# chorowski-lab/pytorch-asr

Hardware: AMD Instinct MI355X
Metric: CTC train-step frames/sec (higher is better)
Workload: dtype bf16; 1 GPU; WSJ mono-char CTC (egs/wsj/yamls/ctc.yaml shapes), DeepSpeech2 conv+4xBiLSTM-320 encoder + FSTDecoder, fwd+bwd+GradientClipping(clip 480000, skip 4.8e+06 = recipe x global_batch/16)+PolyakDecay+Adam, synthetic 40-dim x 1-channel x 1000-frame fbank; batch_per_gpu=768, global_batch=768, frames=1000, classes=49, parallelism=dp1, batch_norm=per-replica statistics, optimizer_steps=139, step_boundary=device: att_speech.fused_step (clip / skip decision + Adam, no read-back)

## Files before the change

### include/asr_amd.h

```cpp
#ifndef ASR_AMD_H
#define ASR_AMD_H

#include <stdint.h>

#ifdef __cplusplus
extern "C" {
#endif

enum {
    ASR_OK = 0,
    ASR_EINVAL = 1,
    ASR_EUNSUPPORTED = 2,
    ASR_ELAUNCH = 3
};

int asr_abi_version(void);

const char *asr_strerror(int code);

int64_t asr_lattice_fwbw_workspace_bytes(int T, int B, int C, int N);

int asr_lattice_fwbw_f32(const float *lp, int T, int B, int C,
                         const int32_t *lens,
                         const int32_t *src_in, const int32_t *il_in,
// ... 169 lines not shown
int64_t asr_conv7x7c32_workspace_bytes(void);
int asr_conv7x7c32_fwd_bf16(const void *x, const float *w, int B, int H, int W, int stride_h,
                            void *y, double *chan_sums, void *workspace, int64_t workspace_bytes,
                            void *stream);
int asr_conv7x7c32_bwd_data_bf16(const void *dy, const float *w, int B, int H, int W,
                                 int stride_h, void *dx, void *workspace,
                                 int64_t workspace_bytes, void *stream);
int asr_conv7x7c32_wgrad_bf16(const void *x, const void *dy, int B, int H, int W, int stride_h,
                              float *dw, void *workspace, int64_t workspace_bytes, void *stream);

int64_t asr_conv1_7x7s2_workspace_bytes(void);
int asr_conv1_7x7s2_fwd(const float *x, const float *w, int B, int T, int F, void *y,
                        double *chan_sums, void *workspace, int64_t workspace_bytes, void *stream);
int asr_conv1_7x7s2_wgrad(const float *x, const void *dy, int B, int T, int F, float *dw,
                          void *workspace, int64_t workspace_bytes, void *stream);

int64_t asr_conv1c_7x7s2_workspace_bytes(int cin);
int asr_conv1c_7x7s2_fwd(const float *x, const float *w, int B, int T, int F, int cin, void *y,
                         double *chan_sums, void *workspace, int64_t workspace_bytes, void *stream);
int asr_conv1c_7x7s2_wgrad(const float *x, const void *dy, int B, int T, int F, int cin,
                           float *dw, void *workspace, int64_t workspace_bytes, void *stream);

int asr_tcn_attention_step_f32(const float *eproj, const float *enc, const int32_t *enc_lens,
                               const float *filt, const float *glob, const float *w_score,
                               float b_score, float temperature,
                               const float *att_prev, const int32_t *parent,
                               int T, int B, int beam, int A, int Kf, int E,
                               float *att_new, float *context, void *stream);

int asr_tcn_attention_scan_fwd_f32(const float *eproj, const float *filt, const float *glob,
// ... 123 lines not shown
```

### pytorch-asr_amd/att_speech/_native.py

```python
import ctypes
import warnings
import os

import torch

_HERE = os.path.dirname(os.path.abspath(__file__))
LIB_PATH = os.environ.get(
    'ASR_AMD_LIB', os.path.join(os.path.dirname(_HERE), 'csrc', 'libasr_amd.so'))

ASR_OK, ASR_EINVAL, ASR_EUNSUPPORTED, ASR_ELAUNCH = 0, 1, 2, 3
ABI_VERSION = 24

_lib = None
EVENT_HOOK = None
_WARNED = {}

_vp, _i, _i64, _f = ctypes.c_void_p, ctypes.c_int, ctypes.c_int64, ctypes.c_float

_SIGNATURES = {
    'asr_abi_version': (ctypes.c_int, []),
    'asr_strerror': (ctypes.c_char_p, [_i]),
    'asr_lattice_fwbw_workspace_bytes': (_i64, [_i, _i, _i, _i]),
    'asr_lattice_fwbw_f32': (_i, [_vp, _i, _i, _i, _vp, _vp, _vp, _vp, _vp, _vp,
                                  _vp, _vp, _i, _i, _i, _i, _f, _vp, _vp, _vp,
# ... 9 lines not shown
    'asr_lattice_viterbi_workspace_bytes': (_i64, [_i, _i, _i]),
    'asr_lattice_forward_f32': (_i, [_vp, _i, _i, _i, _vp, _vp, _vp, _vp, _vp,
                                     _i, _i, _i, _f, _i, _vp, _vp, _vp, _i64,
                                     _vp]),
    'asr_log_softmax_fwd_f32': (_i, [_vp, _i64, _i, _vp, _vp]),
    'asr_log_softmax_bwd_f32': (_i, [_vp, _vp, _i64, _i, _vp, _vp]),
    'asr_sub_rowmax_f32': (_i, [_vp, _i, _i, _i, _vp, _vp, _vp, _vp, _vp]),
    'asr_argmax_rows_f32': (_i, [_vp, _i64, _i, _vp, _vp]),
    'asr_conv7x7c32_workspace_bytes': (_i64, []),
    'asr_conv7x7c32_fwd_bf16': (_i, [_vp, _vp, _i, _i, _i, _i, _vp, _vp, _vp, _i64, _vp]),
    'asr_conv7x7c32_bwd_data_bf16': (_i, [_vp, _vp, _i, _i, _i, _i, _vp, _vp, _i64, _vp]),
    'asr_conv7x7c32_wgrad_bf16': (_i, [_vp, _vp, _i, _i, _i, _i, _vp, _vp, _i64, _vp]),
    'asr_conv1_7x7s2_workspace_bytes': (_i64, []),
    'asr_conv1_7x7s2_fwd': (_i, [_vp, _vp, _i, _i, _i, _vp, _vp, _vp, _i64, _vp]),
    'asr_conv1_7x7s2_wgrad': (_i, [_vp, _vp, _i, _i, _i, _vp, _vp, _i64, _vp]),
    'asr_conv1c_7x7s2_workspace_bytes': (_i64, [_i]),
    'asr_conv1c_7x7s2_fwd': (_i, [_vp, _vp, _i, _i, _i, _i, _vp, _vp, _vp, _i64, _vp]),
    'asr_conv1c_7x7s2_wgrad': (_i, [_vp, _vp, _i, _i, _i, _i, _vp, _vp, _i64, _vp]),
    'asr_log_softmax_shift_fwd_f32': (_i, [_vp, _i, _i, _i, _vp, _vp, _vp, _vp, _vp]),
    'asr_log_softmax_shift_bwd_f32': (_i, [_vp, _vp, _vp, _i64, _i, _vp, _vp]),
    'asr_sum_leading_f32': (_i, [_vp, _i, _i64, _vp, _vp]),
    'asr_adam_chunk_elems': (_i, []),
    'asr_grad_sumsq_partials_f32': (_i, [_vp, _i64, _vp, _i, _vp]),
    'asr_adam_clip_step_f32': (_i, [_vp, _i, _vp, _vp, _vp, _vp, _i, _vp, _f, _f, _f, _f, _f, _f, _f,
                                    _vp, _vp, _vp, _vp]),
    'asr_adam_clip_step_ex_f32': (_i, [_vp, _i, _vp, _vp, _vp, _vp, _i, _vp, _f, _f, _f, _f, _f, _f, _f,
                                       _vp, _vp, _vp, _vp, _vp]),
    'asr_nonfinite_flag_f32': (_i, [_vp, _i, _vp, _vp]),
    'asr_noise_chunk_elems': (_i, []),
    'asr_gaussian_noise_f32': (_i, [_vp, _i, ctypes.c_uint64, ctypes.c_uint32, ctypes.c_uint64, _i, _i, _vp]),
# ... 1120 lines not shown
    if cin == 1:
        nbytes = L.asr_conv1_7x7s2_workspace_bytes()
        ws = torch.empty(nbytes, dtype=torch.uint8, device=x.device)
        check(L.asr_conv1_7x7s2_wgrad(_p(x), _p(dy), B, T, F, _p(dw), _p(ws), nbytes, _stream()),
              'asr_conv1_7x7s2_wgrad')
    else:
        nbytes = L.asr_conv1c_7x7s2_workspace_bytes(cin)
        if nbytes < 0:
            raise NotImplementedError('conv1_wgrad: %d input channels' % cin)
        ws = torch.empty(nbytes, dtype=torch.uint8, device=x.device)
        check(L.asr_conv1c_7x7s2_wgrad(_p(x), _p(dy), B, T, F, cin, _p(dw), _p(ws), nbytes, _stream()),
              'asr_conv1c_7x7s2_wgrad')
    return dw


def split_bf16(x, hi=None, lo=None):
    x = _dev(x, torch.float32, 'x')
    if hi is None:
        hi = torch.empty(x.shape, dtype=torch.bfloat16, device=x.device)
        lo = torch.empty(x.shape, dtype=torch.bfloat16, device=x.device)
        rows, cols, ldx, ldh, ldl = 1, x.numel(), x.numel(), x.numel(), x.numel()
    else:
        if x.dim() != 2 or hi.shape != x.shape or lo.shape != x.shape or x.stride(1) != 1 \
                or hi.stride(1) != 1 or lo.stride(1) != 1 or hi.dtype != torch.bfloat16 or lo.dtype != torch.bfloat16:
            raise ValueError('split_bf16: x, hi, lo must be [rows, cols] with a dense last dimension')
        rows, cols = x.shape
        ldx, ldh, ldl = x.stride(0), hi.stride(0), lo.stride(0)
    check(lib().asr_split_bf16_f32(_p(x), rows, cols, ldx, _p(hi), ldh, _p(lo), ldl, _stream()),
          'asr_split_bf16_f32')
    return hi, lo
# ... 65 lines not shown
```

### pytorch-asr_amd/att_speech/modules/encoders/deep_speech_2.py

```python
import warnings
from collections import OrderedDict

import torch
from torch import nn

from att_speech.modules.encoders.base_encoder import BaseEncoder
from att_speech.modules.encoders.encoder_utils import (
    BatchRNN, Normalization, SequentialWithOptionalAttributes)


class DeepSpeech2(BaseEncoder):
    def __init__(self, sample_batch, conv_normalization='batch_norm',
                 conv_strides=[[2, 2], [2, 1]],
                 conv_kernel_sizes=[[41, 11], [21, 11]],
                 conv_num_features=[32, 32],
                 rnn_hidden_size=768, rnn_nb_layers=5, rnn_projection_size=0,
                 rnn_type=nn.LSTM, rnn_dropout=0.0, rnn_residual=False,
                 rnn_normalization='batch_norm', rnn_subsample=None, **kwargs):
        super(DeepSpeech2, self).__init__(**kwargs)
        import os
        self.conv_bf16 = os.environ.get('ASR_CONV_BF16', '1') != '0'
        self.fused_bn = os.environ.get('ASR_FUSED_BN', '1') != '0'
        self.native_conv = os.environ.get('ASR_NATIVE_CONV', '1') != '0'
        if isinstance(rnn_type, str):
# ... 76 lines not shown
                                            c.dilation, c.groups)
            y = nn.functional.conv2d(
                x.to(torch.bfloat16), c.weight.to(torch.bfloat16),
                None if bias is None else bias.to(torch.bfloat16),
                c.stride, c.padding, c.dilation, c.groups)
            return y if keep_bf16 else y.float()

        def second_conv(x, with_bias=True):
            return run_conv(c2, x, with_bias)

        if fused:
            from att_speech.modules.encoders.native_bn import bn_hardtanh
            from att_speech.modules.encoders import native_conv
            c1 = conv[0]
            sums1 = sums2 = None
            if bf16 and self.native_conv and native_conv.first_supported(c1, features):
                x, sums1 = native_conv.conv1(features, c1)
            else:
                if bf16 and self.native_conv and not getattr(self, '_warned_conv1', False):
                    self._warned_conv1 = True
                    warnings.warn('DeepSpeech2: the first convolution is not a (1 or 3)->32 7x7 stride-(1,2) '
                                  'shape on gradient-free features csrc/conv.hip is built for; using '
                                  'torch / MIOpen for it')
                x = run_conv(c1, features, with_bias=False, keep_bf16=True)
            x = bn_hardtanh(x, conv[1].batch_norm, conv[2], out_bf16=bf16, conv_bias=c1.bias,
                            chan_sums=sums1)
            if bf16 and self.native_conv and native_conv.supported(c2, x):
                y2, sums2 = native_conv.conv7x7c32(x, c2)
            else:
                if bf16 and self.native_conv and not getattr(self, '_warned_conv', False):
                    self._warned_conv = True
                    warnings.warn('DeepSpeech2: the second convolution is not the 32->32 7x7 '
                                  'stride-(3,1) shape csrc/conv.hip is built for; using torch / MIOpen')
                y2 = run_conv(c2, x, with_bias=False, keep_bf16=True)
            x = bn_hardtanh(y2, conv[4].batch_norm, conv[5], time_major=True, conv_bias=c2.bias,
                            chan_sums=sums2, out_bf16=bf16 and self._rnn_takes_bf16(y2))
            return x.view(x.size(0), x.size(1), -1)
        if bf16:
            x = conv[5](conv[4](second_conv(conv[2](conv[1](conv[0](features))))))
        else:
            x = conv(features)
# ... 24 lines not shown
```

### pytorch-asr_amd/att_speech/modules/encoders/native_bn.py

```python
import torch
import torch.distributed as dist

from att_speech import _native

SYNC = {'on': False, 'group': None}


def _sync_active():
    return (SYNC['on'] and dist.is_available() and dist.is_initialized()
            and dist.get_world_size(SYNC['group']) > 1)


def _allreduce_sums(sums, n_local):
    buf = torch.cat([sums.reshape(-1), sums.new_tensor([n_local])])
    dist.all_reduce(buf, op=dist.ReduceOp.SUM, group=SYNC['group'])
    sums.copy_(buf[:-1].view_as(sums))
    return float(buf[-1])


class BNHardtanhFunction(torch.autograd.Function):
    @staticmethod
    def forward(ctx, x, gamma, beta, conv_bias, running_mean, running_var, training, momentum,
                eps, lo, hi, out_bf16, time_major, chan_sums=None, sync_counts=None):
        out, mean, invstd = _native.bn_act_fwd(
            x, gamma.detach(), beta.detach(), running_mean, running_var, training, momentum,
            eps, lo, hi, out_bf16=out_bf16, time_major=time_major,
            conv_bias=None if conv_bias is None else conv_bias.detach(), chan_sums=chan_sums)
        if sync_counts is not None and running_var is not None and momentum:
            nl, nt = sync_counts
            var = invstd.double().pow(-2) - eps
            running_var.add_((momentum * var * (nt / (nt - 1.0) - nl / (nl - 1.0))).float())
        ctx.has_cb = conv_bias is not None
        ctx.save_for_backward(x, gamma, beta, mean, invstd,
                              conv_bias if conv_bias is not None else gamma)
        ctx.cfg = (training, lo, hi, time_major)
        ctx.sync = training and _sync_active()
        return out

    @staticmethod
    def backward(ctx, dy):
        x, gamma, beta, mean, invstd, cb = ctx.saved_tensors
        training, lo, hi, time_major = ctx.cfg
        dx, dgamma, dbeta, dcb = _native.bn_act_bwd(
            x, gamma.detach(), beta.detach(), mean, invstd, training, lo, hi, dy,
            time_major=time_major, conv_bias=cb.detach() if ctx.has_cb else None,
            sync=_allreduce_sums if ctx.sync else None)
        return (dx, dgamma, dbeta, dcb) + (None,) * 11


def bn_hardtanh(x, bn, act, out_bf16=False, time_major=False, conv_bias=None, chan_sums=None):
    use_batch_stats = bn.training or bn.running_mean is None
    momentum = 0.0
    rm = rv = None
    if use_batch_stats and bn.training and bn.track_running_stats and bn.running_mean is not None:
        bn.num_batches_tracked.add_(1)
        momentum = bn.momentum if bn.momentum is not None else 1.0 / float(bn.num_batches_tracked)
        rm, rv = bn.running_mean, bn.running_var
    elif not use_batch_stats:
        rm, rv = bn.running_mean, bn.running_var
    if x.dtype != torch.bfloat16:
        x = x.float()
    sync_counts = None
    if use_batch_stats and bn.training and _sync_active():
        n_local = float(x.shape[0] * x.shape[2] * x.shape[3])
        if chan_sums is None:
            xd = x.double()
            chan_sums = torch.stack([xd.sum((0, 2, 3)), (xd * xd).sum((0, 2, 3))])
        else:
            chan_sums = chan_sums.clone()
        n_total = _allreduce_sums(chan_sums, n_local)
        chan_sums.mul_(n_local / n_total)
        sync_counts = (n_local, n_total)
    return BNHardtanhFunction.apply(x, bn.weight, bn.bias, conv_bias, rm, rv, use_batch_stats,
                                    momentum, bn.eps, float(act.min_val), float(act.max_val),
                                    out_bf16, time_major, chan_sums if use_batch_stats else None,
                                    sync_counts)
```

### pytorch-asr_amd/att_speech/modules/encoders/native_conv.py

```python
import torch

from att_speech import _native


def supported(conv, x):
    return (x.is_cuda and isinstance(conv, torch.nn.Conv2d) and conv.in_channels == 32
            and conv.out_channels == 32 and tuple(conv.kernel_size) == (7, 7)
            and tuple(conv.stride) == (3, 1) and tuple(conv.padding) == (0, 0)
            and tuple(conv.dilation) == (1, 1) and conv.groups == 1
            and x.dim() == 4 and x.size(2) >= 7 and 7 <= x.size(3) <= 48)


class Conv7x7C32Function(torch.autograd.Function):
    @staticmethod
    def forward(ctx, x, weight):
        x = x.to(torch.bfloat16).contiguous(memory_format=torch.channels_last)
        ctx.save_for_backward(x, weight)
        y, sums = _native.conv7x7c32_fwd(x, weight.detach(), 3, want_sums=True)
        ctx.mark_non_differentiable(sums)
        return y, sums

    @staticmethod
    def backward(ctx, dy, _dsums):
        x, weight = ctx.saved_tensors
        dx = dw = None
# ... 18 lines not shown

    @staticmethod
    def forward(ctx, x, weight):
        x = x.float().contiguous()
        ctx.save_for_backward(x, weight)
        y, sums = _native.conv1_fwd(x, weight.detach(), want_sums=True)
        ctx.mark_non_differentiable(sums)
        return y, sums

    @staticmethod
    def backward(ctx, dy, _dsums):
        x, weight = ctx.saved_tensors
        return None, (_native.conv1_wgrad(x, dy) if ctx.needs_input_grad[1] else None)


def conv1(features, conv):
    if features.size(1) == 1:
        return Conv1Function.apply(features[:, 0], conv.weight)
    return Conv1Function.apply(features.permute(0, 2, 3, 1), conv.weight)


def conv7x7c32(x, conv):
    return Conv7x7C32Function.apply(x, conv.weight)
```

### pytorch-asr_amd/csrc/bnact.hip

```cpp
#include "common.h"
#include "../../include/asr_amd.h"

namespace {

using namespace asr;

struct BnParams {
    const float *x;
    int B, C, HW, Wd;
    const float *gamma, *beta;
    const float *mean, *invstd;
    const float *shift;
    float lo, hi;
};

__global__ __launch_bounds__(256) void bn_stats_kernel(const float *x, const float *shift, int C, int HW, double *sums) {
    __shared__ float red[64];
    const int c = blockIdx.x, b = blockIdx.y;
    const float *p = x + ((size_t)b * C + c) * HW;
    const float sh0 = shift ? shift[c] : 0.f;
    float s = 0.f, q = 0.f;
    for (int i = threadIdx.x; i < HW; i += 256) {
        const float v = p[i] + sh0;
        s += v;
// ... 390 lines not shown
    const int C = p.C;
    NHWC8_THREAD_SETUP(p.P);
    float m[8], is[8], g[8], be[8], k1[8], k2[8], s[8], q[8];
#pragma unroll
    for (int i = 0; i < 8; ++i) {
        m[i] = p.mean[c0 + i] - (p.shift ? p.shift[c0 + i] : 0.f);
        is[i] = p.invstd[c0 + i]; g[i] = p.gamma[c0 + i]; be[i] = p.beta[c0 + i];
        k1[i] = MODE == 1 && training ? (float)(sums[2 * (c0 + i)] / n) : 0.f;
        k2[i] = MODE == 1 && training ? (float)(sums[2 * (c0 + i) + 1] / n) : 0.f;
        s[i] = q[i] = 0.f;
    }
    auto one = [&](int64_t pix, const F8 &v, const F8 &dv) {
        F8 o;
#pragma unroll
        for (int i = 0; i < 8; ++i) {
            const float xh = (v.v[i] - m[i]) * is[i];
            const float y = fmaf(xh, g[i], be[i]);
            const float d = (y > p.lo && y < p.hi) ? dv.v[i] : 0.f;
            if (MODE == 0) { s[i] += d; q[i] += d * xh; }
            else o.v[i] = g[i] * is[i] * (d - k1[i] - xh * k2[i]);
        }
        if (MODE == 1) store8(dx + pix * C + c0, o);
    };
    for (int64_t pix = (int64_t)blockIdx.x * 2 * PL + pl; pix < pend; pix += cstep) {
        if (pix + PL < pend) {
            const F8 v0 = load8(px + pix * C + c0), v1 = load8(px + (pix + PL) * C + c0);
            const F8 d0 = load8(dy + pix * C + c0), d1 = load8(dy + (pix + PL) * C + c0);
            one(pix, v0, d0);
            one(pix + PL, v1, d1);
        } else {
            one(pix, load8(px + pix * C + c0), load8(dy + pix * C + c0));
        }
    }
    if (MODE == 0) nhwc_block_atomics8(s, q, C, sums);
}
// ... 207 lines not shown
    return hipGetLastError() == hipSuccess ? ASR_OK : ASR_ELAUNCH;
}

extern "C" int asr_bn_act_bwd_phase_f32(const void *x, int x_bf16, const float *conv_bias, int B, int C, int H, int W,
                                  const float *gamma, const float *beta,
                                  const float *save_mean, const float *save_invstd,
                                  int channels_last,
                                  int training, float lo, float hi,
                                  const void *dy, int dy_bf16, int dy_time_major,
                                  void *dx, float *dgamma, float *dbeta, float *dconv_bias,
                                  void *workspace, int64_t workspace_bytes, int phase,
                                  double n_total, void *stream) {
    if (phase < 0 || phase > 2 || (phase == 2 && !(n_total >= 1.0))) return ASR_EINVAL;
    const bool do_reduce = phase != 2, do_apply = phase != 1;
    if (bad_shape(B, C, H, W) || !x || !gamma || !beta || !save_mean || !save_invstd || !dy ||
        !dx || !dgamma || !dbeta)
        return ASR_EINVAL;
    if (!workspace || workspace_bytes < asr_bn_act_workspace_bytes(C)) return ASR_EINVAL;
    hipStream_t s = (hipStream_t)stream;
    double *sums = (double *)workspace;
    const int HW = H * W;
    const dim3 grid(C, B);
    BnParams p;
    p.x = (const float *)x; p.B = B; p.C = C; p.HW = HW; p.Wd = W; p.gamma = gamma; p.beta = beta;
    p.mean = save_mean; p.invstd = save_invstd; p.shift = conv_bias; p.lo = lo; p.hi = hi;
    const double n = phase == 2 ? n_total : (double)B * HW;
    if (do_reduce)
        hipLaunchKernelGGL(zero_doubles_kernel, dim3((2 * C + 255) / 256), dim3(256), 0, s, sums, 2 * C);
    if (x_bf16 && !channels_last) return ASR_EUNSUPPORTED;
    if (channels_last) {
        if (C % 4 != 0 || C > 1024 || 256 % (C / 4) != 0) return ASR_EUNSUPPORTED;
// ... 91 lines not shown
```

### pytorch-asr_amd/csrc/conv.hip

```cpp
#include <type_traits>
#include "common.h"
#include "../../include/asr_amd.h"

namespace {

typedef __attribute__((ext_vector_type(8))) __bf16 bf16x8;
typedef __attribute__((ext_vector_type(16))) float f32x16;
typedef __attribute__((ext_vector_type(4))) unsigned int u32x4;
typedef __attribute__((ext_vector_type(4))) float f32x4;
typedef __attribute__((ext_vector_type(4))) __bf16 bf16x4;

constexpr int CH = 32;
constexpr int KS = 7;
constexpr int PIX = 80;
constexpr int KSTEPS = KS * KS * CH / 16;

typedef __attribute__((ext_vector_type(4))) int rsrc_words;
__device__ __forceinline__ rsrc_words conv_raw_rsrc(const void *base, unsigned bytes) {
    const unsigned long long a = (unsigned long long)base;
    rsrc_words r;
    r.x = __builtin_amdgcn_readfirstlane((int)(unsigned)a);
    r.y = __builtin_amdgcn_readfirstlane((int)((unsigned)(a >> 32) & 0xffffu));
    r.z = __builtin_amdgcn_readfirstlane((int)bytes);
    r.w = 0x00020000;
    return r;
// ... 715 lines not shown
                                        16 * g + 8 * (lane >> 5)) = o4;
        }
    }
    __syncthreads();
    const int rows_here = (p.To - t0) < C1_ROWS ? (p.To - t0) : C1_ROWS;
    char *yb = reinterpret_cast<char *>(p.y) + ((size_t)b * p.To + t0) * Fo * 64;
    for (int c = tid; c < rows_here * Fo * 4; c += 256)
        *reinterpret_cast<u32x4 *>(yb + (size_t)c * 16) =
            *reinterpret_cast<const u32x4 *>(reinterpret_cast<const char *>(oimg) + (size_t)c * 16);
    if (p.partial)
        chan_partial_sums(oimg, rows_here * Fo, reinterpret_cast<float *>(oimg + (size_t)ntiles * 32 * CH),
                          p.partial + ((size_t)blockIdx.y * gridDim.x + blockIdx.x) * 64);
}

constexpr int C1_WGS = 1024;
template <int DI, int WPT>
__global__ __launch_bounds__(256) void conv1_wgrad_kernel(Conv1Params p) {
    extern __shared__ char smem[];
    const int tid = threadIdx.x, lane = tid & 63;
    const int wave = __builtin_amdgcn_readfirstlane(tid >> 6);
    const int Fo = p.Fo, npix = C1_ROWS * Fo, nks = npix >> 4;
    const int nwin = (C1_ROWS + 8) * Fo;
    char *wimg = smem;
    char *dimg = smem + (size_t)nwin * 16;
    f32x16 acc[2];
#pragma unroll
    for (int t = 0; t < 2; ++t)
#pragma unroll
        for (int j = 0; j < 16; ++j) acc[t][j] = 0.f;
    const int h = lane >> 5, q = (lane & 15) >> 2, pp = lane & 3, chalf = (lane >> 4) & 1;
    const unsigned a_off = (unsigned)((8 * h + q) * PIX + (16 * chalf + 4 * pp) * 2);
    const int ktl = 2 * chalf + (pp >> 1);
    const unsigned b_lane = (unsigned)(8 * (pp & 1));
    const int chunks_per_utt = (p.To + C1_ROWS - 1) / C1_ROWS;
    const int nchunks = p.B * chunks_per_utt;
    const unsigned fmagic = (1u << 20) / (unsigned)Fo + 1u;
    u32x4 dreg[DI];
    float2 wreg[WPT][4];
    auto fetch = [&](int c) {
        const int b = c / chunks_per_utt, t0 = (c - b * chunks_per_utt) * C1_ROWS;
        const char *yb = reinterpret_cast<const char *>(p.y) + ((size_t)b * p.To + t0) * Fo * 64;
        const int rows_here = (p.To - t0) < C1_ROWS ? (p.To - t0) : C1_ROWS;
#pragma unroll
        for (int k = 0; k < DI; ++k) {
            const int i = tid + 256 * k, pix = i >> 2;
            dreg[k] = pix < rows_here * Fo ? *reinterpret_cast<const u32x4 *>(yb + (size_t)i * 16) : u32x4{0u, 0u, 0u, 0u};
        }
        const float *xb = p.x + (size_t)b * p.T * p.F;
#pragma unroll
        for (int u = 0; u < WPT; ++u) {
            const unsigned i = (unsigned)(tid + 256 * u);
            const unsigned row = (i * fmagic) >> 20, fo = i - row * (unsigned)Fo;
            const int t = t0 - 6 + (int)row;
            const bool ok = (int)i < nwin && t >= 0 && t < p.T;
            const float2 *src = reinterpret_cast<const float2 *>(xb + (size_t)(ok ? t : 0) * p.F + 2 * fo);
#pragma unroll
            for (int j = 0; j < 4; ++j) wreg[u][j] = ok ? src[j] : float2{0.f, 0.f};
        }
    };
    auto stash = [&]() {
#pragma unroll
        for (int k = 0; k < DI; ++k) {
            const int i = tid + 256 * k, pix = i >> 2, part = i & 3;
            if (pix < npix) *reinterpret_cast<u32x4 *>(dimg + pix * PIX + part * 16) = dreg[k];
        }
#pragma unroll
        for (int u = 0; u < WPT; ++u) {
            const int i = tid + 256 * u;
            bf16x8 v;
#pragma unroll
            for (int j = 0; j < 4; ++j) { v[2 * j] = (__bf16)wreg[u][j].x; v[2 * j + 1] = (__bf16)wreg[u][j].y; }
            if (i < nwin) *reinterpret_cast<bf16x8 *>(wimg + (size_t)i * 16) = v;
        }
    };
    if ((int)blockIdx.x < nchunks) fetch(blockIdx.x);
    for (int c = blockIdx.x; c < nchunks; c += gridDim.x) {
        __syncthreads();
        stash();
        __syncthreads();
        if (c + (int)gridDim.x < nchunks) fetch(c + gridDim.x);
        for (int ks = wave; ks < nks; ks += 4) {
            const bf16x8 a = tr_frag(dimg + (size_t)(16 * ks) * PIX + a_off);
            const unsigned p0 = (unsigned)(16 * ks + 8 * h + q), p1 = p0 + 4;
            const unsigned r0 = (p0 * fmagic) >> 20, f0 = p0 - r0 * (unsigned)Fo;
            const unsigned r1 = (p1 * fmagic) >> 20, f1 = p1 - r1 * (unsigned)Fo;
#pragma unroll
            for (int nt = 0; nt < 2; ++nt) {
                const int kt = 4 * nt + ktl;
                const s16x4 lo = __builtin_amdgcn_ds_read_tr16_b64_v4i16(
                    (lds_s16x4 *)(wimg + (size_t)((r0 + kt) * Fo + f0) * 16 + b_lane));
                const s16x4 hi = __builtin_amdgcn_ds_read_tr16_b64_v4i16(
                    (lds_s16x4 *)(wimg + (size_t)((r1 + kt) * Fo + f1) * 16 + b_lane));
                s16x8 v;
                v.s0 = lo.x; v.s1 = lo.y; v.s2 = lo.z; v.s3 = lo.w;
                v.s4 = hi.x; v.s5 = hi.y; v.s6 = hi.z; v.s7 = hi.w;
                acc[nt] = __builtin_amdgcn_mfma_f32_32x32x16_bf16(a, __builtin_bit_cast(bf16x8, v), acc[nt], 0, 0, 0);
            }
        }
    }
    __syncthreads();
    float *red = reinterpret_cast<float *>(smem);
#pragma unroll
    for (int nt = 0; nt < 2; ++nt)
#pragma unroll
        for (int j = 0; j < 16; ++j) red[((wave * 2 + nt) * 16 + j) * 64 + lane] = acc[nt][j];
    __syncthreads();
    float *out = p.partial + (size_t)blockIdx.x * 2 * 1024;
    for (int e = tid; e < 2 * 1024; e += 256)
        out[e] = red[e] + red[2048 + e] + red[4096 + e] + red[6144 + e];
}

__global__ __launch_bounds__(1024) void conv1_wgrad_reduce_kernel(const float *partial, int nparts, float *dw) {
    __shared__ float lds4[1024];
    const float s = partial_sum(partial, nparts, 2 * 1024, lds4);
    const int e = blockIdx.x * 64 + (threadIdx.x & 63);
    if (threadIdx.x >= 64) return;
    const int nt = e >> 10, j = (e >> 6) & 15, l = e & 63;
    const int co = (j & 3) + 8 * (j >> 2) + 4 * (l >> 5), tap = 32 * nt + (l & 31);
    const int kt = tap >> 3, kf = tap & 7;
    if (kt < KS && kf < KS) dw[(co * KS + kt) * KS + kf] = s;
}


template <int CIN>
// ... 415 lines not shown
    const dim3 grid((To + C1_ROWS - 1) / C1_ROWS, B);
    p.partial = chan_sums ? (float *)((char *)workspace + 4 * 64 * 8 * 2) : nullptr;
    if (chan_sums && (int64_t)grid.x * grid.y * 64 * 4 > asr_conv1_7x7s2_workspace_bytes() - 4 * 64 * 8 * 2 - 256)
        return ASR_EUNSUPPORTED;
    const int ntiles = (C1_ROWS * Fo + 31) / 32;
    const size_t lds = (size_t)(C1_ROWS + 8) * Fo * 16 + (size_t)ntiles * 32 * CH * 2 + 512 * 4;
    if (lds > 64 * 1024) return ASR_EUNSUPPORTED;
    hipLaunchKernelGGL(conv1_fwd_kernel, grid, dim3(256), lds, s, p);
    if (chan_sums) {
        hipLaunchKernelGGL(zero_chan_sums_kernel, dim3(1), dim3(64), 0, s, chan_sums);
        hipLaunchKernelGGL(chan_sums_reduce_kernel, dim3(64), dim3(1024), 0, s, p.partial, (int)(grid.x * grid.y), chan_sums);
    }
    return hipGetLastError() == hipSuccess ? ASR_OK : ASR_ELAUNCH;
}

extern "C" int asr_conv1_7x7s2_wgrad(const float *x, const void *dy, int B, int T, int F,
                                     float *dw, void *workspace, int64_t workspace_bytes,
                                     void *stream) {
    int To, Fo;
    const int rc = conv1_shapes(B, T, F, &To, &Fo);
    if (rc != ASR_OK) return rc;
    if (!x || !dy || !dw || !workspace || workspace_bytes < asr_conv1_7x7s2_workspace_bytes())
        return ASR_EINVAL;
    hipStream_t s = (hipStream_t)stream;
    Conv1Params p;
    p.x = x; p.wpack = nullptr; p.y = (__bf16 *)const_cast<void *>(dy);
    p.partial = (float *)((char *)workspace + 4 * 64 * 8 * 2);
    p.B = B; p.T = T; p.F = F; p.To = To; p.Fo = Fo;
    size_t lds = (size_t)(C1_ROWS + 8) * Fo * 16 + (size_t)C1_ROWS * Fo * PIX;
    if (lds < 4 * 2 * 1024 * 4) lds = 4 * 2 * 1024 * 4;
    if (lds > 64 * 1024) return ASR_EUNSUPPORTED;
    const int chunks = B * ((To + C1_ROWS - 1) / C1_ROWS);
    const int nwg = chunks < C1_WGS ? chunks : C1_WGS;
    const int di = (C1_ROWS * Fo * 4 + 255) / 256, wpt = ((C1_ROWS + 8) * Fo + 255) / 256;
    void (*kern)(Conv1Params) = di <= 5 && wpt <= 2 ? conv1_wgrad_kernel<5, 2>
                              : (di <= 8 && wpt <= 3 ? conv1_wgrad_kernel<8, 3> : conv1_wgrad_kernel<16, 6>);
    hipLaunchKernelGGL(kern, dim3(nwg), dim3(256), lds, s, p);
    hipLaunchKernelGGL(conv1_wgrad_reduce_kernel, dim3(2 * 1024 / 64), dim3(1024), 0, s, p.partial, nwg, dw);
    return hipGetLastError() == hipSuccess ? ASR_OK : ASR_ELAUNCH;
}


extern "C" int64_t asr_conv1c_7x7s2_workspace_bytes(int cin) {
    if (cin != 3) return -1;
    const int64_t wg = (int64_t)C1_WGS * 2 * cin * 1024 * 4, cs = (int64_t)(1 << 17) * 64 * 4;
    return (int64_t)cin * 4 * 64 * 8 * 2 + (wg > cs ? wg : cs) + 256;
}

extern "C" int asr_conv1c_7x7s2_fwd(const float *x, const float *w, int B, int T, int F, int cin, void *y,
                                    double *chan_sums, void *workspace, int64_t workspace_bytes,
                                    void *stream) {
    int To, Fo;
    const int rc = conv1_shapes(B, T, F, &To, &Fo);
    if (rc != ASR_OK) return rc;
// ... 62 lines not shown
```

Measured before the change: 37.05 million frames/s.

## Fuse first-layer BN+hardtanh backward into conv1 weight-gradient kernel

```diff
diff --git a/include/asr_amd.h b/include/asr_amd.h
--- a/include/asr_amd.h
+++ b/include/asr_amd.h
@@ -207,6 +207,11 @@
                         double *chan_sums, void *workspace, int64_t workspace_bytes, void *stream);
 int asr_conv1_7x7s2_wgrad(const float *x, const void *dy, int B, int T, int F, float *dw,
                           void *workspace, int64_t workspace_bytes, void *stream);
+int asr_conv1_7x7s2_wgrad_bn(const float *x, const void *d_act, const void *x1, int B, int T, int F,
+                             const float *mean, const float *invstd, const float *gamma,
+                             const float *beta, const float *conv_bias, float lo, float hi,
+                             int training, double n, const double *sums, float *dw,
+                             void *workspace, int64_t workspace_bytes, void *stream);
 
 int64_t asr_conv1c_7x7s2_workspace_bytes(int cin);
 int asr_conv1c_7x7s2_fwd(const float *x, const float *w, int B, int T, int F, int cin, void *y,
diff --git a/pytorch-asr_amd/att_speech/_native.py b/pytorch-asr_amd/att_speech/_native.py
--- a/pytorch-asr_amd/att_speech/_native.py
+++ b/pytorch-asr_amd/att_speech/_native.py
@@ -47,6 +47,8 @@
     'asr_conv1_7x7s2_workspace_bytes': (_i64, []),
     'asr_conv1_7x7s2_fwd': (_i, [_vp, _vp, _i, _i, _i, _vp, _vp, _vp, _i64, _vp]),
     'asr_conv1_7x7s2_wgrad': (_i, [_vp, _vp, _i, _i, _i, _vp, _vp, _i64, _vp]),
+    'asr_conv1_7x7s2_wgrad_bn': (_i, [_vp, _vp, _vp, _i, _i, _i, _vp, _vp, _vp, _vp, _vp, _f, _f, _i,
+                                      ctypes.c_double, _vp, _vp, _vp, _i64, _vp]),
     'asr_conv1c_7x7s2_workspace_bytes': (_i64, [_i]),
     'asr_conv1c_7x7s2_fwd': (_i, [_vp, _vp, _i, _i, _i, _i, _vp, _vp, _vp, _i64, _vp]),
     'asr_conv1c_7x7s2_wgrad': (_i, [_vp, _vp, _i, _i, _i, _i, _vp, _vp, _i64, _vp]),
@@ -1197,6 +1199,45 @@
     return dw
 
 
+def conv1_bn_bwd(x, x1, gamma, beta, mean, invstd, training, lo, hi, d_act, conv_bias=None,
+                 sync=None, want_dw=True):
+    x = _dev(x, torch.float32, 'x')
+    x1, B, C, H, W = _nhwc_bf16(x1, 'x1')
+    d_act = _nhwc_bf16(d_act, 'd_act')[0]
+    if x.dim() != 3 or C != 32 or tuple(d_act.shape) != tuple(x1.shape) \
+            or (B, H, W) != (x.shape[0], x.shape[1] + 6, (x.shape[2] - 7) // 2 + 1):
+        raise ValueError('conv1_bn_bwd: x [B, T, F], x1 / d_act [B, 32, T + 6, (F - 7) // 2 + 1]')
+    gamma, beta = _dev(gamma, torch.float32, 'gamma'), _dev(beta, torch.float32, 'beta')
+    L = lib()
+    dev = x.device
+    dgamma = torch.empty(C, dtype=torch.float32, device=dev)
+    dbeta = torch.empty(C, dtype=torch.float32, device=dev)
+    dcb = None
+    if conv_bias is not None:
+        conv_bias = _dev(conv_bias, torch.float32, 'conv_bias')
+        dcb = torch.empty(C, dtype=torch.float32, device=dev)
+    nb = L.asr_bn_act_workspace_bytes(C)
+    bws = torch.empty(nb, dtype=torch.uint8, device=dev)
+    training = bool(training)
+    check(L.asr_bn_act_bwd_phase_f32(
+        _p(x1), 1, _p(conv_bias), B, C, H, W, _p(gamma), _p(beta), _p(mean), _p(invstd), 1,
+        int(training), float(lo), float(hi), _p(d_act), 1, 0, None, _p(dgamma), _p(dbeta), _p(dcb),
+        _p(bws), nb, 1, 0.0, _stream()), 'asr_bn_act_bwd_phase_f32')
+    if not want_dw:
+        return None, dgamma, dbeta, dcb
+    n = float(B) * H * W
+    if sync is not None and training:
+        n = sync(bws[:2 * C * 8].view(torch.float64), n)
+    dw = torch.empty((32, 1, 7, 7), dtype=torch.float32, device=dev)
+    nbytes = L.asr_conv1_7x7s2_workspace_bytes()
+    ws = torch.empty(nbytes, dtype=torch.uint8, device=dev)
+    check(L.asr_conv1_7x7s2_wgrad_bn(
+        _p(x), _p(d_act), _p(x1), x.shape[0], x.shape[1], x.shape[2], _p(mean), _p(invstd),
+        _p(gamma), _p(beta), _p(conv_bias), float(lo), float(hi), int(training), float(n), _p(bws),
+        _p(dw), _p(ws), nbytes, _stream()), 'asr_conv1_7x7s2_wgrad_bn')
+    return dw, dgamma, dbeta, dcb
+
+
 def split_bf16(x, hi=None, lo=None):
     x = _dev(x, torch.float32, 'x')
     if hi is None:
diff --git a/pytorch-asr_amd/att_speech/modules/encoders/deep_speech_2.py b/pytorch-asr_amd/att_speech/modules/encoders/deep_speech_2.py
--- a/pytorch-asr_amd/att_speech/modules/encoders/deep_speech_2.py
+++ b/pytorch-asr_amd/att_speech/modules/encoders/deep_speech_2.py
@@ -114,7 +114,11 @@
             from att_speech.modules.encoders import native_conv
             c1 = conv[0]
             sums1 = sums2 = None
-            if bf16 and self.native_conv and native_conv.first_supported(c1, features):
+            native1 = bf16 and self.native_conv and native_conv.first_supported(c1, features)
+            fused1 = native1 and native_conv.fused_bn_bwd(c1, c2, features)
+            if fused1:
+                x = native_conv.conv1_bn_hardtanh(features, c1, conv[1].batch_norm, conv[2])
+            elif native1:
                 x, sums1 = native_conv.conv1(features, c1)
             else:
                 if bf16 and self.native_conv and not getattr(self, '_warned_conv1', False):
@@ -123,8 +127,9 @@
                                   'shape on gradient-free features csrc/conv.hip is built for; using '
                                   'torch / MIOpen for it')
                 x = run_conv(c1, features, with_bias=False, keep_bf16=True)
-            x = bn_hardtanh(x, conv[1].batch_norm, conv[2], out_bf16=bf16, conv_bias=c1.bias,
-                            chan_sums=sums1)
+            if not fused1:
+                x = bn_hardtanh(x, conv[1].batch_norm, conv[2], out_bf16=bf16, conv_bias=c1.bias,
+                                chan_sums=sums1)
             if bf16 and self.native_conv and native_conv.supported(c2, x):
                 y2, sums2 = native_conv.conv7x7c32(x, c2)
             else:
diff --git a/pytorch-asr_amd/att_speech/modules/encoders/native_bn.py b/pytorch-asr_amd/att_speech/modules/encoders/native_bn.py
--- a/pytorch-asr_amd/att_speech/modules/encoders/native_bn.py
+++ b/pytorch-asr_amd/att_speech/modules/encoders/native_bn.py
@@ -27,9 +27,7 @@
             eps, lo, hi, out_bf16=out_bf16, time_major=time_major,
             conv_bias=None if conv_bias is None else conv_bias.detach(), chan_sums=chan_sums)
         if sync_counts is not None and running_var is not None and momentum:
-            nl, nt = sync_counts
-            var = invstd.double().pow(-2) - eps
-            running_var.add_((momentum * var * (nt / (nt - 1.0) - nl / (nl - 1.0))).float())
+            fix_running_var(running_var, invstd, momentum, eps, sync_counts)
         ctx.has_cb = conv_bias is not None
         ctx.save_for_backward(x, gamma, beta, mean, invstd,
                               conv_bias if conv_bias is not None else gamma)
@@ -48,7 +46,7 @@
         return (dx, dgamma, dbeta, dcb) + (None,) * 11
 
 
-def bn_hardtanh(x, bn, act, out_bf16=False, time_major=False, conv_bias=None, chan_sums=None):
+def bn_mode(x, bn, chan_sums):
     use_batch_stats = bn.training or bn.running_mean is None
     momentum = 0.0
     rm = rv = None
@@ -58,8 +56,6 @@
         rm, rv = bn.running_mean, bn.running_var
     elif not use_batch_stats:
         rm, rv = bn.running_mean, bn.running_var
-    if x.dtype != torch.bfloat16:
-        x = x.float()
     sync_counts = None
     if use_batch_stats and bn.training and _sync_active():
         n_local = float(x.shape[0] * x.shape[2] * x.shape[3])
@@ -71,7 +67,19 @@
         n_total = _allreduce_sums(chan_sums, n_local)
         chan_sums.mul_(n_local / n_total)
         sync_counts = (n_local, n_total)
+    return rm, rv, use_batch_stats, momentum, chan_sums if use_batch_stats else None, sync_counts
+
+
+def fix_running_var(running_var, invstd, momentum, eps, sync_counts):
+    nl, nt = sync_counts
+    var = invstd.double().pow(-2) - eps
+    running_var.add_((momentum * var * (nt / (nt - 1.0) - nl / (nl - 1.0))).float())
+
+
+def bn_hardtanh(x, bn, act, out_bf16=False, time_major=False, conv_bias=None, chan_sums=None):
+    if x.dtype != torch.bfloat16:
+        x = x.float()
+    rm, rv, use_batch_stats, momentum, chan_sums, sync_counts = bn_mode(x, bn, chan_sums)
     return BNHardtanhFunction.apply(x, bn.weight, bn.bias, conv_bias, rm, rv, use_batch_stats,
                                     momentum, bn.eps, float(act.min_val), float(act.max_val),
-                                    out_bf16, time_major, chan_sums if use_batch_stats else None,
-                                    sync_counts)
+                                    out_bf16, time_major, chan_sums, sync_counts)
diff --git a/pytorch-asr_amd/att_speech/modules/encoders/native_conv.py b/pytorch-asr_amd/att_speech/modules/encoders/native_conv.py
--- a/pytorch-asr_amd/att_speech/modules/encoders/native_conv.py
+++ b/pytorch-asr_amd/att_speech/modules/encoders/native_conv.py
@@ -3,12 +3,16 @@
 from att_speech import _native
 
 
-def supported(conv, x):
-    return (x.is_cuda and isinstance(conv, torch.nn.Conv2d) and conv.in_channels == 32
+def supported_shape(conv, H, W):
+    return (isinstance(conv, torch.nn.Conv2d) and conv.in_channels == 32
             and conv.out_channels == 32 and tuple(conv.kernel_size) == (7, 7)
             and tuple(conv.stride) == (3, 1) and tuple(conv.padding) == (0, 0)
             and tuple(conv.dilation) == (1, 1) and conv.groups == 1
-            and x.dim() == 4 and x.size(2) >= 7 and 7 <= x.size(3) <= 48)
+            and H >= 7 and 7 <= W <= 48)
+
+
+def supported(conv, x):
+    return x.is_cuda and x.dim() == 4 and supported_shape(conv, x.size(2), x.size(3))
 
 
 class Conv7x7C32Function(torch.autograd.Function):
@@ -57,6 +61,51 @@
         return None, (_native.conv1_wgrad(x, dy) if ctx.needs_input_grad[1] else None)
 
 
+class Conv1BNHardtanhFunction(torch.autograd.Function):
+
+    @staticmethod
+    def forward(ctx, x, weight, gamma, beta, conv_bias, bn, lo, hi):
+        from att_speech.modules.encoders import native_bn
+        x = x.float().contiguous()
+        x1, sums = _native.conv1_fwd(x, weight.detach(), want_sums=True)
+        rm, rv, training, momentum, sums, sync_counts = native_bn.bn_mode(x1, bn, sums)
+        cb = None if conv_bias is None else conv_bias.detach()
+        out, mean, invstd = _native.bn_act_fwd(
+            x1, gamma.detach(), beta.detach(), rm, rv, training, momentum, bn.eps, lo, hi,
+            out_bf16=True, conv_bias=cb, chan_sums=sums)
+        if sync_counts is not None and rv is not None and momentum:
+            native_bn.fix_running_var(rv, invstd, momentum, bn.eps, sync_counts)
+        ctx.has_cb = conv_bias is not None
+        ctx.save_for_backward(x, x1, gamma, beta, mean, invstd,
+                              conv_bias if conv_bias is not None else gamma)
+        ctx.cfg = (training, lo, hi, training and native_bn._sync_active())
+        return out
+
+    @staticmethod
+    def backward(ctx, dy):
+        from att_speech.modules.encoders import native_bn
+        x, x1, gamma, beta, mean, invstd, cb = ctx.saved_tensors
+        training, lo, hi, sync = ctx.cfg
+        if not any(ctx.needs_input_grad[1:5]):
+            return (None,) * 8
+        dw, dgamma, dbeta, dcb = _native.conv1_bn_bwd(
+            x, x1, gamma.detach(), beta.detach(), mean, invstd, training, lo, hi, dy,
+            conv_bias=cb.detach() if ctx.has_cb else None,
+            sync=native_bn._allreduce_sums if sync else None, want_dw=ctx.needs_input_grad[1])
+        return None, dw, dgamma, dbeta, dcb, None, None, None
+
+
+def fused_bn_bwd(conv1, conv2, features):
+    import os
+    return (os.environ.get('ASR_CONV1_BN_BWD', '1') != '0' and features.size(1) == 1
+            and supported_shape(conv2, features.size(2) + 6, (features.size(3) - 7) // 2 + 1))
+
+
+def conv1_bn_hardtanh(features, conv, bn, act):
+    return Conv1BNHardtanhFunction.apply(features[:, 0], conv.weight, bn.weight, bn.bias, conv.bias,
+                                         bn, float(act.min_val), float(act.max_val))
+
+
 def conv1(features, conv):
     if features.size(1) == 1:
         return Conv1Function.apply(features[:, 0], conv.weight)
diff --git a/pytorch-asr_amd/csrc/bnact.hip b/pytorch-asr_amd/csrc/bnact.hip
--- a/pytorch-asr_amd/csrc/bnact.hip
+++ b/pytorch-asr_amd/csrc/bnact.hip
@@ -1,4 +1,5 @@
 #include "common.h"
+#include "bnact_elem.h"
 #include "../../include/asr_amd.h"
 
 namespace {
@@ -428,11 +429,11 @@
         F8 o;
 #pragma unroll
         for (int i = 0; i < 8; ++i) {
-            const float xh = (v.v[i] - m[i]) * is[i];
-            const float y = fmaf(xh, g[i], be[i]);
-            const float d = (y > p.lo && y < p.hi) ? dv.v[i] : 0.f;
+            float xh, d;
+            const float r = bn_act_bwd_elem(v.v[i], dv.v[i], m[i], is[i], g[i], be[i], k1[i], k2[i],
+                                            p.lo, p.hi, xh, d);
             if (MODE == 0) { s[i] += d; q[i] += d * xh; }
-            else o.v[i] = g[i] * is[i] * (d - k1[i] - xh * k2[i]);
+            else o.v[i] = r;
         }
         if (MODE == 1) store8(dx + pix * C + c0, o);
     };
@@ -670,7 +671,7 @@
     if (phase < 0 || phase > 2 || (phase == 2 && !(n_total >= 1.0))) return ASR_EINVAL;
     const bool do_reduce = phase != 2, do_apply = phase != 1;
     if (bad_shape(B, C, H, W) || !x || !gamma || !beta || !save_mean || !save_invstd || !dy ||
-        !dx || !dgamma || !dbeta)
+        (do_apply && !dx) || !dgamma || !dbeta)
         return ASR_EINVAL;
     if (!workspace || workspace_bytes < asr_bn_act_workspace_bytes(C)) return ASR_EINVAL;
     hipStream_t s = (hipStream_t)stream;
diff --git a/pytorch-asr_amd/csrc/bnact_elem.h b/pytorch-asr_amd/csrc/bnact_elem.h
--- /dev/null
+++ b/pytorch-asr_amd/csrc/bnact_elem.h
@@ -0,0 +1,15 @@
+#pragma once
+#include <hip/hip_runtime.h>
+
+namespace asr {
+
+__device__ __forceinline__ float bn_act_bwd_elem(float v, float dv, float m, float is, float g, float be,
+                                                 float k1, float k2, float lo, float hi, float &xh,
+                                                 float &d) {
+    xh = (v - m) * is;
+    const float y = fmaf(xh, g, be);
+    d = (y > lo && y < hi) ? dv : 0.f;
+    return g * is * (d - k1 - xh * k2);
+}
+
+}
diff --git a/pytorch-asr_amd/csrc/conv.hip b/pytorch-asr_amd/csrc/conv.hip
--- a/pytorch-asr_amd/csrc/conv.hip
+++ b/pytorch-asr_amd/csrc/conv.hip
@@ -1,5 +1,6 @@
 #include <type_traits>
 #include "common.h"
+#include "bnact_elem.h"
 #include "../../include/asr_amd.h"
 
 namespace {
@@ -9,6 +10,7 @@
 typedef __attribute__((ext_vector_type(4))) unsigned int u32x4;
 typedef __attribute__((ext_vector_type(4))) float f32x4;
 typedef __attribute__((ext_vector_type(4))) __bf16 bf16x4;
+typedef __attribute__((ext_vector_type(2))) __bf16 bf16x2;
 
 constexpr int CH = 32;
 constexpr int KS = 7;
@@ -754,8 +756,18 @@
 }
 
 constexpr int C1_WGS = 1024;
-template <int DI, int WPT>
-__global__ __launch_bounds__(256) void conv1_wgrad_kernel(Conv1Params p) {
+struct Conv1Bn {
+    const __bf16 *x1;
+    const float *mean, *invstd, *gamma, *beta, *shift;
+    const double *sums;
+    double n;
+    float lo, hi;
+    int training;
+    int nvirt;
+};
+
+template <int DI, int WPT, bool BN>
+__device__ __forceinline__ void conv1_wgrad_body(const Conv1Params &p, const Conv1Bn &bn) {
     extern __shared__ char smem[];
     const int tid = threadIdx.x, lane = tid & 63;
     const int wave = __builtin_amdgcn_readfirstlane(tid >> 6);
@@ -763,11 +775,18 @@
     const int nwin = (C1_ROWS + 8) * Fo;
     char *wimg = smem;
     char *dimg = smem + (size_t)nwin * 16;
+    const size_t img_bytes = (size_t)nwin * 16 + (size_t)npix * PIX;
+    float *cst = reinterpret_cast<float *>(smem + (img_bytes < 4 * 2 * 1024 * 4 ? 4 * 2 * 1024 * 4 : img_bytes));
+    if (BN && tid < CH) {
+        const int c = tid;
+        cst[8 * c + 0] = bn.mean[c] - (bn.shift ? bn.shift[c] : 0.f);
+        cst[8 * c + 1] = bn.invstd[c];
+        cst[8 * c + 2] = bn.gamma[c];
+        cst[8 * c + 3] = bn.beta[c];
+        cst[8 * c + 4] = bn.training ? (float)(bn.sums[2 * c] / bn.n) : 0.f;
+        cst[8 * c + 5] = bn.training ? (float)(bn.sums[2 * c + 1] / bn.n) : 0.f;
+    }
     f32x16 acc[2];
-#pragma unroll
-    for (int t = 0; t < 2; ++t)
-#pragma unroll
-        for (int j = 0; j < 16; ++j) acc[t][j] = 0.f;
     const int h = lane >> 5, q = (lane & 15) >> 2, pp = lane & 3, chalf = (lane >> 4) & 1;
     const unsigned a_off = (unsigned)((8 * h + q) * PIX + (16 * chalf + 4 * pp) * 2);
     const int ktl = 2 * chalf + (pp >> 1);
@@ -775,16 +794,21 @@
     const int chunks_per_utt = (p.To + C1_ROWS - 1) / C1_ROWS;
     const int nchunks = p.B * chunks_per_utt;
     const unsigned fmagic = (1u << 20) / (unsigned)Fo + 1u;
-    u32x4 dreg[DI];
+    u32x4 dreg[DI], xreg[BN ? DI : 1];
     float2 wreg[WPT][4];
     auto fetch = [&](int c) {
         const int b = c / chunks_per_utt, t0 = (c - b * chunks_per_utt) * C1_ROWS;
         const char *yb = reinterpret_cast<const char *>(p.y) + ((size_t)b * p.To + t0) * Fo * 64;
+        const char *x1b = reinterpret_cast<const char *>(bn.x1) + ((size_t)b * p.To + t0) * Fo * 64;
         const int rows_here = (p.To - t0) < C1_ROWS ? (p.To - t0) : C1_ROWS;
 #pragma unroll
         for (int k = 0; k < DI; ++k) {
             const int i = tid + 256 * k, pix = i >> 2;
             dreg[k] = pix < rows_here * Fo ? *reinterpret_cast<const u32x4 *>(yb + (size_t)i * 16) : u32x4{0u, 0u, 0u, 0u};
+            if (BN)
+                xreg[k] = pix < rows_here * Fo
+                              ? *reinterpret_cast<const u32x4 *>(x1b + (size_t)i * 16)
+                              : u32x4{0u, 0u, 0u, 0u};
         }
         const float *xb = p.x + (size_t)b * p.T * p.F;
 #pragma unroll
@@ -798,11 +822,37 @@
             for (int j = 0; j < 4; ++j) wreg[u][j] = ok ? src[j] : float2{0.f, 0.f};
         }
     };
-    auto stash = [&]() {
+    auto stash = [&](int c) {
+        int nvalid = npix;
+        if (BN) {
+            const int t0 = (c % chunks_per_utt) * C1_ROWS;
+            nvalid = ((p.To - t0) < C1_ROWS ? (p.To - t0) : C1_ROWS) * Fo;
+            const float *cc = cst + 8 * (8 * (tid & 3));
+#pragma unroll
+            for (int jp = 0; jp < 4; ++jp) {
+                asm volatile("" ::: "memory");
+                const f32x4 a0 = *reinterpret_cast<const f32x4 *>(cc + 16 * jp);
+                const f32x4 b0 = *reinterpret_cast<const f32x4 *>(cc + 16 * jp + 4);
+                const f32x4 a1 = *reinterpret_cast<const f32x4 *>(cc + 16 * jp + 8);
+                const f32x4 b1 = *reinterpret_cast<const f32x4 *>(cc + 16 * jp + 12);
+#pragma unroll
+                for (int k = 0; k < DI; ++k) {
+                    const unsigned dw = dreg[k][jp], xw = xreg[k][jp];
+                    float xh, d;
+                    const float o0 = asr::bn_act_bwd_elem(__builtin_bit_cast(float, xw << 16), __builtin_bit_cast(float, dw << 16),
+                                                          a0[0], a0[1], a0[2], a0[3], b0[0], b0[1], bn.lo, bn.hi, xh, d);
+                    const float o1 = asr::bn_act_bwd_elem(__builtin_bit_cast(float, xw & 0xffff0000u), __builtin_bit_cast(float, dw & 0xffff0000u),
+                                                          a1[0], a1[1], a1[2], a1[3], b1[0], b1[1], bn.lo, bn.hi, xh, d);
+                    const bf16x2 o = {(__bf16)o0, (__bf16)o1};
+                    dreg[k][jp] = __builtin_bit_cast(unsigned, o);
+                }
+            }
+        }
 #pragma unroll
         for (int k = 0; k < DI; ++k) {
             const int i = tid + 256 * k, pix = i >> 2, part = i & 3;
-            if (pix < npix) *reinterpret_cast<u32x4 *>(dimg + pix * PIX + part * 16) = dreg[k];
+            if (pix < npix) *reinterpret_cast<u32x4 *>(dimg + pix * PIX + part * 16) =
+                (!BN || pix < nvalid) ? dreg[k] : u32x4{0u, 0u, 0u, 0u};
         }
 #pragma unroll
         for (int u = 0; u < WPT; ++u) {
@@ -813,12 +863,19 @@
             if (i < nwin) *reinterpret_cast<bf16x8 *>(wimg + (size_t)i * 16) = v;
         }
     };
-    if ((int)blockIdx.x < nchunks) fetch(blockIdx.x);
-    for (int c = blockIdx.x; c < nchunks; c += gridDim.x) {
-        __syncthreads();
-        stash();
-        __syncthreads();
-        if (c + (int)gridDim.x < nchunks) fetch(c + gridDim.x);
+    const int nv = BN ? bn.nvirt : (int)gridDim.x;
+    int v = blockIdx.x;
+    do {
+#pragma unroll
+    for (int t = 0; t < 2; ++t)
+#pragma unroll
+        for (int j = 0; j < 16; ++j) acc[t][j] = 0.f;
+    if (v < nchunks) fetch(v);
+    for (int c = v; c < nchunks; c += nv) {
+        __syncthreads();
+        stash(c);
+        __syncthreads();
+        if (c + nv < nchunks) fetch(c + nv);
         for (int ks = wave; ks < nks; ks += 4) {
             const bf16x8 a = tr_frag(dimg + (size_t)(16 * ks) * PIX + a_off);
             const unsigned p0 = (unsigned)(16 * ks + 8 * h + q), p1 = p0 + 4;
@@ -845,9 +902,19 @@
 #pragma unroll
         for (int j = 0; j < 16; ++j) red[((wave * 2 + nt) * 16 + j) * 64 + lane] = acc[nt][j];
     __syncthreads();
-    float *out = p.partial + (size_t)blockIdx.x * 2 * 1024;
+    float *out = p.partial + (size_t)v * 2 * 1024;
     for (int e = tid; e < 2 * 1024; e += 256)
         out[e] = red[e] + red[2048 + e] + red[4096 + e] + red[6144 + e];
+    } while (BN && (v += (int)gridDim.x) < nv);
+}
+
+template <int DI, int WPT>
+__global__ __launch_bounds__(256) void conv1_wgrad_kernel(Conv1Params p) {
+    conv1_wgrad_body<DI, WPT, false>(p, Conv1Bn{});
+}
+template <int DI, int WPT, int WPE>
+__global__ __launch_bounds__(256, WPE) void conv1_wgrad_bn_kernel(Conv1Params p, Conv1Bn bn) {
+    conv1_wgrad_body<DI, WPT, true>(p, bn);
 }
 
 __global__ __launch_bounds__(1024) void conv1_wgrad_reduce_kernel(const float *partial, int nparts, float *dw) {
@@ -1293,9 +1360,9 @@
     return hipGetLastError() == hipSuccess ? ASR_OK : ASR_ELAUNCH;
 }
 
-extern "C" int asr_conv1_7x7s2_wgrad(const float *x, const void *dy, int B, int T, int F,
-                                     float *dw, void *workspace, int64_t workspace_bytes,
-                                     void *stream) {
+static int conv1_wgrad_launch(const float *x, const void *dy, int B, int T, int F, float *dw,
+                              void *workspace, int64_t workspace_bytes, const Conv1Bn *bn,
+                              void *stream) {
     int To, Fo;
     const int rc = conv1_shapes(B, T, F, &To, &Fo);
     if (rc != ASR_OK) return rc;
@@ -1312,11 +1379,48 @@
     const int chunks = B * ((To + C1_ROWS - 1) / C1_ROWS);
     const int nwg = chunks < C1_WGS ? chunks : C1_WGS;
     const int di = (C1_ROWS * Fo * 4 + 255) / 256, wpt = ((C1_ROWS + 8) * Fo + 255) / 256;
-    void (*kern)(Conv1Params) = di <= 5 && wpt <= 2 ? conv1_wgrad_kernel<5, 2>
-                              : (di <= 8 && wpt <= 3 ? conv1_wgrad_kernel<8, 3> : conv1_wgrad_kernel<16, 6>);
-    hipLaunchKernelGGL(kern, dim3(nwg), dim3(256), lds, s, p);
+    const int size = di <= 5 && wpt <= 2 ? 0 : (di <= 8 && wpt <= 3 ? 1 : 2);
+    if (bn) {
+        void (*kern)(Conv1Params, Conv1Bn) =
+            size == 0 ? conv1_wgrad_bn_kernel<5, 2, 2>
+                      : (size == 1 ? conv1_wgrad_bn_kernel<8, 3, 2> : conv1_wgrad_bn_kernel<16, 6, 1>);
+        const int per_cu = size == 2 ? 1 : 2;
+        Conv1Bn b = *bn;
+        b.nvirt = nwg;
+        const int grid = nwg > 256 * per_cu ? 256 * per_cu : nwg;
+        lds += CH * 8 * 4;
+        if (lds > 64 * 1024 &&
+            hipFuncSetAttribute((const void *)kern, hipFuncAttributeMaxDynamicSharedMemorySize, (int)lds) != hipSuccess)
+            return ASR_EUNSUPPORTED;
+        hipLaunchKernelGGL(kern, dim3(grid), dim3(256), lds, s, p, b);
+    } else {
+        void (*kern)(Conv1Params) = size == 0 ? conv1_wgrad_kernel<5, 2>
+                                  : (size == 1 ? conv1_wgrad_kernel<8, 3> : conv1_wgrad_kernel<16, 6>);
+        hipLaunchKernelGGL(kern, dim3(nwg), dim3(256), lds, s, p);
+    }
     hipLaunchKernelGGL(conv1_wgrad_reduce_kernel, dim3(2 * 1024 / 64), dim3(1024), 0, s, p.partial, nwg, dw);
     return hipGetLastError() == hipSuccess ? ASR_OK : ASR_ELAUNCH;
+}
+
+extern "C" int asr_conv1_7x7s2_wgrad(const float *x, const void *dy, int B, int T, int F,
+                                     float *dw, void *workspace, int64_t workspace_bytes,
+                                     void *stream) {
+    return conv1_wgrad_launch(x, dy, B, T, F, dw, workspace, workspace_bytes, nullptr, stream);
+}
+
+extern "C" int asr_conv1_7x7s2_wgrad_bn(const float *x, const void *d_act, const void *x1, int B, int T,
+                                        int F, const float *mean, const float *invstd,
+                                        const float *gamma, const float *beta, const float *conv_bias,
+                                        float lo, float hi, int training, double n, const double *sums,
+                                        float *dw, void *workspace, int64_t workspace_bytes,
+                                        void *stream) {
+    if (!x1 || !mean || !invstd || !gamma || !beta) return ASR_EINVAL;
+    if (training && (!sums || !(n >= 1.0))) return ASR_EINVAL;
+    Conv1Bn bn;
+    bn.x1 = (const __bf16 *)x1; bn.mean = mean; bn.invstd = invstd; bn.gamma = gamma; bn.beta = beta;
+    bn.shift = conv_bias; bn.sums = sums; bn.n = n; bn.lo = lo; bn.hi = hi; bn.training = training;
+    bn.nvirt = 0;
+    return conv1_wgrad_launch(x, d_act, B, T, F, dw, workspace, workspace_bytes, &bn, stream);
 }
 
 
```

Result: faster. 37.54 million frames/s (median of 6 runs) (+1.3%).
